# moonmath-ai/LiteAttention

Measured on AMD Instinct MI355X. Metric: self-attn TFLOPS + ms/step @ seq=75k d=128 bf16, sparsity 0->77%; 1/2/4/8 GPU, higher is better.
Workload: dtype bf16; 1 GPU; QK-Skip self-attention fwd, B=1 S=75600 H=40 D=128 bf16, imposed 42% sparsity (banded lists, thr=-inf), tiles 256x64; parallelism=heads sharded 1x40, launcher=single process

## Files before the change

### liteattention_amd/csrc/gen_blocks.py

```python
from gen_asm import *


def flush_block(flush_label, back_label, T, tail=None):
    label(flush_label)
    flush_domask(T[4], T[5])
    emit(f"s_add_u32 {s(S_DOWORD)}, {s(S_DOWORD)}, 4")
    emit(f"s_mov_b32 {s(S_BIT)}, 1")
    if tail:
        tail()
    else:
        emit("s_waitcnt lgkmcnt(0)")
    emit(f"s_branch {back_label}")


def inval_block(lbl, back, R):
    label(lbl)
    for qb in R.QBS:
        emit(f"v_mov_b32 {v(R.MLOC[qb])}, {v(R.NEGINF)}")
        emit(f"v_mov_b32 {v(R.NMS[qb])}, {v(R.NEGINF)}")
    emit(f"s_branch {back}")


def rescale_o_block(lbl, back, T, scaled, nops=2, tail=None):
    label(lbl)
# ... 96 lines not shown
    emit(f"s_cmp_eq_u32 {s(S_DOMASK)}, 0")
    emit(f"s_cbranch_scc1 {nofl}")
    flush_domask(T[4], T[5])
    label(nofl)
    for _ in range(nops):
        emit("s_nop 15")


def q_row_address(T, row):
    emit(f"v_min_i32 {v(T[3])}, {v(row)}, {s(S_T1)}")
    emit(f"v_mad_u64_u32 {vr(T[4], 2)}, {sr(S_T64)}, {v(T[3])}, {s(S_QRS)}, 0")
    emit(f"v_add_co_u32 {v(T[4])}, vcc, {v(T[4])}, {v(T[6])}")
    emit(f"v_addc_co_u32 {v(T[5])}, vcc, 0, {v(T[5])}, vcc")
    emit(f"v_add_co_u32 {v(T[4])}, vcc, {s(S_QBASE)}, {v(T[4])}")
    emit(f"v_mov_b32 {v(T[7])}, {s(S_QBASE + 1)}")
    emit(f"v_addc_co_u32 {v(T[5])}, vcc, {v(T[5])}, {v(T[7])}, vcc")


def q_rows_to_agprs(T, n_qb, n_frag, frag_bytes, q_a0, row_of, loaded=None):
    emit(f"v_lshlrev_b32 {v(T[6])}, 4, {v(T[0])}")
    for qb in range(n_qb):
        q_row_address(T, row_of(qb, False))
        for f in range(n_frag):
            emit(f"global_load_dwordx4 {vr(4 * n_frag * qb + 4 * f, 4)}, {vr(T[4], 2)}, off offset:{frag_bytes * f}")
    (loaded or (lambda: emit("s_waitcnt vmcnt(0)")))()
    for qb in range(n_qb):
        emit(f"v_cmp_gt_i32 vcc, {s(S_SEQLENQ)}, {v(row_of(qb, True))}")
        for r in range(4 * n_frag * qb, 4 * n_frag * (qb + 1)):
            emit(f"v_cndmask_b32 {v(r)}, 0, {v(r)}, vcc")
    for r in range(4 * n_frag * n_qb):
        emit(f"v_accvgpr_write_b32 a{q_a0 + r}, {v(r)}")


def zero_accumulators(regs):
    emit("; ---- state")
    for r in regs:
        emit(f"v_accvgpr_write_b32 a{r}, 0")


def read_tile_table(T, TABV):
    emit("; ---- tile addresses of positions 1..3 from the table; K(0) fragments -> AGPRs, S(0) = K(0) Q^T, then K(1) fragments")
    emit(f"v_mov_b32 {v(T[6])}, {s(S_TAB)}")
    emit(f"ds_read_b64 {vr(T[8], 2)}, {v(T[6])} offset:32")
    emit(f"ds_read_b64 {vr(T[10], 2)}, {v(T[6])} offset:48")
    emit(f"ds_read_b64 {vr(T[12], 2)}, {v(T[6])} offset:24")
    emit(f"v_add_u32 {v(TABV)}, 32, {v(T[6])}")


def k2_base(T):
    emit(("DRAIN",))
    emit(f"v_readfirstlane_b32 {s(TBS[0])}, {v(T[8])}")
    emit(f"v_readfirstlane_b32 {s(TBS[0] + 1)}, {v(T[9])}")


def stage_k2(k_ops, T):
    for it in k_ops:
        out.append(it)
        if "m0" in it:
            emit("s_nop 0")
    for dst, src in ((TBS[0], T[10]), (TBS[0] + 1, T[11]), (VBS[0], T[12]), (VBS[0] + 1, T[13])):
        emit(f"v_readfirstlane_b32 {s(dst)}, {v(src)}")


def mask_ops(T, NEGINF, lane_key, keys):
    for key, regs in keys:
        emit(f"v_add_u32 {v(T[0])}, {key}, {v(lane_key)}")
# ... 14 lines not shown
```

### liteattention_amd/csrc/gen_fwd_x64.py

```python
#!/usr/bin/env python
import os
import sys
from types import SimpleNamespace

from gen_asm import *
from gen_blocks import *
from gen_epilogue import store_epilogue

set_label_prefix(".LX")
OPT = options("LA_X64_OPT")
SCHEDULE_ONLY = {"snake", "x", "cap1", "cap2", "dmagaps", "dmapol", "align", "pad4", "pad4b", "e64", "wp2", "wp2b", "wc2", "kearly", "klate", "klate2", "expblock", "norot", "w2", "pk"}


DTYPE = os.environ.get("LA_X64_DTYPE", "bf16")
MFMA_OP = {"bf16": "v_mfma_f32_32x32x16_bf16", "f16": "v_mfma_f32_32x32x16_f16"}[DTYPE]
CVT_OP = {"bf16": "v_cvt_pk_bf16_f32", "f16": "v_cvt_pk_f16_f32"}[DTYPE]
W2 = "w2" in OPT
D = int(os.environ.get("LA_X64_D", "128"))
assert D in (64, 96, 128, 192, 256)
assert not W2 or D == 64
HALF = os.environ.get("LA_X64_FORM", "") == "half"
assert not HALF or (D in (64, 96, 128) and not W2)
DL = 64 if D == 64 else (128 if D <= 128 else 256)
NQB = 1 if W2 else (2 if DL <= 128 else 1)
# ... 656 lines not shown
        emit("s_waitcnt lgkmcnt(0)")
        w2_qk()
        w2_stats(first_tile=False, can_be_first=False)
        label(skip)
    w2_tail()


def prologue():
    stamp(0)
    read_params(LANE, T[0], [S_HSTRIDE] if HALF else [])
    if HALF:
        emit("; ---- half = wave >> 1: its vote words, its activity words; the window starts as positions [0, 64)")
        emit(f"s_lshr_b32 {s(S_T0)}, {s(S_WAVE)}, 1")
        emit(f"s_mul_i32 {s(S_T0)}, {s(S_T0)}, {s(S_HSTRIDE)}")
        emit(f"s_add_u32 {s(S_DOFLAGS)}, {s(S_DOFLAGS)}, {s(S_T0)}")
        emit(f"s_add_u32 {s(S_ACTPTR)}, {s(S_EXPORT)}, {s(S_T0)}")
        emit(f"v_mov_b32 {v(T[0])}, {s(S_ACTPTR)}")
        emit(f"ds_read_b64 {vr(T[4], 2)}, {v(T[0])}")
        emit("s_waitcnt lgkmcnt(0)")
        emit(f"v_readfirstlane_b32 {s(S_ACT)}, {v(T[4])}")
        emit(f"v_readfirstlane_b32 {s(S_ACT + 1)}, {v(T[5])}")
        emit(f"s_add_u32 {s(S_ACTPTR)}, {s(S_ACTPTR)}, 4")
    emit(f"s_mov_b32 {s(S_CC)}, {s(S_C)}")
    emit(f"s_mov_b32 {s(S_CC + 1)}, {s(S_C)}")
    emit(f"s_sub_u32 {s(S_NM1)}, {s(S_NTILES)}, 1")
    emit(f"s_lshl_b32 {s(S_DMAW)}, {s(S_WAVE)}, {ROW_SHIFT + (3 if W2 else 4)}")
    emit(f"s_add_u32 {s(S_DMAW)}, {s(S_DMAW)}, {s(S_LDS)}")
    emit(f"s_mov_b32 {s(S_I)}, 0")
    if DOTSUM:
        emit(f"s_mov_b32 {s(S_ONES)}, {ONES_BITS}")
    emit(f"s_mov_b32 {s(S_RESC)}, 0")
    emit(f"v_mov_b32 {v(NEGINF)}, 0xff800000")

    emit("; ---- per-lane constants")
    emit(f"v_lshrrev_b32 {v(T[0])}, 5, {v(LANE)}")
    emit(f"v_lshlrev_b32 {v(HH4)}, 2, {v(T[0])}")
    emit(f"v_and_b32 {v(T[1])}, 31, {v(LANE)}")
    emit(f"v_and_b32 {v(T[2])}, 15, {v(LANE)}")
    emit(f"v_lshlrev_b32 {v(T[3])}, {ROW_SHIFT}, {v(T[1])}")
    emit(f"v_add_u32 {v(T[3])}, {s(S_LDS)}, {v(T[3])}")
    if DL == 64:
        emit(f"v_lshrrev_b32 {v(T[8])}, 1, {v(T[1])}")
        emit(f"v_and_b32 {v(T[8])}, 7, {v(T[8])}")
    for ks in range(4 if DL == 64 else 8):
        emit(f"v_add_u32 {v(T[4])}, {2 * ks}, {v(T[0])}")
        emit(f"v_xor_b32 {v(T[4])}, {v(T[4])}, {v(T[8] if DL == 64 else T[2])}")
        emit(f"v_lshl_add_u32 {v(KADDR[ks])}, {v(T[4])}, 4, {v(T[3])}")
    emit(f"v_lshrrev_b32 {v(T[4])}, 2, {v(T[2])}")
    emit(f"v_add_u32 {v(T[5])}, {v(HH4)}, {v(T[4])}")
    emit(f"v_lshlrev_b32 {v(T[5])}, {ROW_SHIFT}, {v(T[5])}")
    emit(f"v_add_u32 {v(T[5])}, {s(S_LDS)}, {v(T[5])}")
    emit(f"v_add_u32 {v(T[5])}, {V_REGION}, {v(T[5])}")
    emit(f"v_lshrrev_b32 {v(T[6])}, 4, {v(LANE)}")
    emit(f"v_and_b32 {v(T[7])}, 1, {v(T[6])}")
    emit(f"v_lshlrev_b32 {v(T[7])}, 5, {v(T[7])}")
    emit(f"v_and_b32 {v(T[8])}, 3, {v(T[2])}")
    emit(f"v_lshl_or_b32 {v(T[7])}, {v(T[8])}, 3, {v(T[7])}")
    emit(f"v_add_u32 {v(T[5])}, {v(T[5])}, {v(T[7])}")
    if DL == 64:
        emit(f"v_lshrrev_b32 {v(T[4])}, 1, {v(T[4])}")
    for db in range(2 if DL == 64 else 4):
        emit(f"v_xor_b32 {v(T[7])}, {db}, {v(T[4])}")
        emit(f"v_lshl_add_u32 {v(VADDR[db])}, {v(T[7])}, 6, {v(T[5])}")
    emit(f"s_lshl_b32 {s(S_T0)}, {s(S_WAVE)}, {3 if W2 else 4}")
    if DL == 64:
        emit(f"v_lshrrev_b32 {v(T[6])}, 3, {v(LANE)}")
        emit(f"v_and_b32 {v(T[7])}, 7, {v(LANE)}")
        emit(f"v_add_u32 {v(RIPROW)}, {s(S_T0)}, {v(T[6])}")
        emit(f"v_lshrrev_b32 {v(T[8])}, 1, {v(T[6])}")
        emit(f"v_xor_b32 {v(RAGK)}, {v(T[7])}, {v(T[8])}")
        emit(f"v_lshlrev_b32 {v(RAGK)}, 4, {v(RAGK)}")
# ... 15 lines not shown
    else:
        emit(f"v_add_u32 {v(RIPROW)}, {s(S_T0)}, {v(T[0])}")
        emit(f"v_xor_b32 {v(RAGK)}, {v(T[1])}, {v(T[0])}")
        emit(f"v_lshlrev_b32 {v(RAGK)}, 4, {v(RAGK)}")
        emit(f"v_lshlrev_b32 {v(RAGV)}, 2, {v(T[0])}")
        emit(f"v_xor_b32 {v(RAGV)}, {v(T[1])}, {v(RAGV)}")
        emit(f"v_lshlrev_b32 {v(RAGV)}, 4, {v(RAGV)}")
    emit(f"s_mov_b32 {s(S_T1)}, {s(S_LASTROW)}")
    RSTEP = (64 // NW) // PW
    for j in range(PW):
        bias = DMA_BIAS - 1024 * (j & 3)
        emit(f"v_add_u32 {v(T[4])}, {RSTEP * j}, {v(RIPROW)}")
        emit(f"v_min_i32 {v(T[4])}, {v(T[4])}, {s(S_T1)}")
        emit(f"v_mul_lo_u32 {v(LK[j])}, {v(T[4])}, {s(S_KRS)}")
        def in_row(reg):
            if D != DL:
                emit(f"v_subrev_u32 {v(T[7])}, {2 * DL - 2 * D}, {v(reg)}")
                emit(f"v_cmp_le_u32 vcc, {2 * D}, {v(reg)}")
                emit(f"v_cndmask_b32 {v(reg)}, {v(reg)}, {v(T[7])}, vcc")
        emit(f"v_xor_b32 {v(T[5])}, {((RSTEP * j) >> (1 if DL == 64 else 0)) << 4}, {v(RAGK)}")
        in_row(T[5])
        emit(f"v_add_u32 {v(LK[j])}, {v(LK[j])}, {v(T[5])}")
        emit(f"v_mul_lo_u32 {v(LV[j])}, {v(T[4])}, {s(S_VRS)}")
        if D == 128 or D == 64:
            emit(f"v_add_u32 {v(LV[j])}, {v(LV[j])}, {v(RAGV)}")
        else:
            emit(f"v_xor_b32 {v(T[5])}, {((RSTEP * j) & 3) << 6}, {v(RAGV)}")
            in_row(T[5])
            emit(f"v_add_u32 {v(LV[j])}, {v(LV[j])}, {v(T[5])}")
        if bias:
            emit(f"v_add_u32 {v(LK[j])}, {bias}, {v(LK[j])}")
            emit(f"v_add_u32 {v(LV[j])}, {bias}, {v(LV[j])}")

    emit("; ---- Q fragments -> AGPRs: row q_row0 + 64*wave + 32*qb + l31, d = 16*ks + 8*hh; rows past seqlen_q are ZERO rows")
    emit(f"s_lshl_b32 {s(S_T0)}, {s(S_WAVE)}, {5 + NQB - 1}")
    emit(f"s_add_u32 {s(S_T0)}, {s(S_T0)}, {s(S_QROW0)}")
    emit(f"s_sub_u32 {s(S_T1)}, {s(S_SEQLENQ)}, 1")

    def q_row(qb, again):
        if not again:
            emit(f"v_add_u32 {v(QROW[qb])}, {s(S_T0)}, {v(T[1])}")
            if qb:
                emit(f"v_add_u32 {v(QROW[qb])}, 32, {v(QROW[qb])}")
        return QROW[qb]
    q_rows_to_agprs(T, NQB, KS, 32, Q_A0, q_row, loaded=lambda: (stamp(1), emit("s_waitcnt vmcnt(0)"), stamp(2)))
    zero_accumulators(range(16 * DB * NQB))
    for qb in range(NQB):
        emit(f"v_mov_b32 {v(MTRUE[qb])}, 0xff800000")
        emit(f"v_mov_b32 {v(L0[qb])}, 0")
        emit(f"v_mov_b32 {v(L1[qb])}, 0")
        emit(f"v_mov_b32 {v(ALPHA[qb])}, 1.0")
        if HALF:
            emit(f"v_mov_b32 {v(MREF[qb])}, 0xff800000")
            emit(f"v_mov_b32 {v(MTHR[qb])}, 0xff800000")
            emit(f"v_mov_b32 {v(NMS[qb])}, 0")

    if W2:
        emit("; ---- w2: K(0) fragments -> AGPRs")
        emit(f"v_mov_b32 {v(TABV)}, {s(S_TAB)}")
        emit(f"v_add_u32 {v(TABV)}, 16, {v(TABV)}")
        for j in range(NKF):
            emit(k_read(0, j))
        emit(f"s_mov_b32 {s(S_DOMASK)}, 0")
        emit(f"s_mov_b32 {s(S_BIT)}, 1")
        emit(f"s_mov_b32 {s(S_DOWORD)}, {s(S_DOFLAGS)}")
        emit(("DRAIN",))
        emit("s_barrier")
        return
    read_tile_table(T, TABV)
    for j in range(NKF):
        emit(k_read(0, j))
    k2_base(T)
    ord1 = [(f & 1) * KS + (f >> 1) for f in range(NKF)]
    if HALF:
        noqk0 = new_label("noqk0")
        emit(f"s_bitcmp1_b32 {s(S_ACT)}, 0")
        emit(f"s_cbranch_scc0 {noqk0}")
    for t in range(NG):
        out.append(mfma_qk(0, ord1[t // NQB], qb_of(t)))
    if HALF:
        label(noqk0)
    for j in range(NKF):
        emit(k_read(KV_TILE, j))
    emit(("DRAIN",))
    emit("s_barrier")
    stage_k2(dma_ops(0, 0, do_k=True, do_v=False), T)
    emit("s_nop 7")
    if HALF:
# ... 139 lines not shown
```

### liteattention_amd/csrc/la_fwd_common.h

```cpp
#pragma once
#include <hip/hip_runtime.h>
#include <stdint.h>

#include "la_kernel_params.h"

namespace la {

typedef __bf16 bf16x8 __attribute__((ext_vector_type(8)));
typedef short s16x4 __attribute__((ext_vector_type(4)));
typedef short s16x8 __attribute__((ext_vector_type(8)));
typedef float f32x16 __attribute__((ext_vector_type(16)));
typedef float f32x8 __attribute__((ext_vector_type(8)));
typedef unsigned int u32x2 __attribute__((ext_vector_type(2)));
typedef unsigned int u32x4 __attribute__((ext_vector_type(4)));

typedef _Float16 f16x8 __attribute__((ext_vector_type(8)));
typedef _Float16 f16x4 __attribute__((ext_vector_type(4)));
typedef __bf16 bf16x4 __attribute__((ext_vector_type(4)));
typedef float f32x4 __attribute__((ext_vector_type(4)));

template <bool F16> struct Elem16;
template <> struct Elem16<false> {
    typedef bf16x8 x8;
    typedef bf16x4 x4;
// ... 77 lines not shown
        if (!((live[pos >> 5] >> (pos & 31)) & 1u)) continue;
        const int n = seq[pos];
        const bool raw_skip = !first && !((doflags[pos >> 5] >> (pos & 31)) & 1u);
        first = false;
        bool skip = raw_skip;
        if (has_md && skip) {
            if (md.end > n && md.has_more()) { md.advance(); md.load(k_tiles); }
            const bool must_do = n <= md.start && n > md.end;
            skip = skip && !must_do;
        }
        if (skip != is_skipping) {
            if (w <= k_tiles) write_row[w] = static_cast<ListT>(n);
            ++w;
            is_skipping = skip;
        }
        if ((endflags[pos >> 5] >> (pos & 31)) & 1u) {
            is_skipping = true;
            if (!raw_skip) { if (w <= k_tiles) write_row[w] = static_cast<ListT>(n); ++w; }
        }
    }
    write_row[0] = static_cast<ListT>(min(w - 1, k_tiles));
}

__device__ __forceinline__ int wave_inclusive_scan(int v) {
    v += __builtin_amdgcn_update_dpp(0, v, 0x111, 0xf, 0xf, true);
    v += __builtin_amdgcn_update_dpp(0, v, 0x112, 0xf, 0xf, true);
    v += __builtin_amdgcn_update_dpp(0, v, 0x114, 0xf, 0xf, true);
    v += __builtin_amdgcn_update_dpp(0, v, 0x118, 0xf, 0xf, true);
    v += __builtin_amdgcn_update_dpp(0, v, 0x142, 0xa, 0xf, false);
    v += __builtin_amdgcn_update_dpp(0, v, 0x143, 0xc, 0xf, false);
    return v;
}

template <typename ListT>
__device__ __forceinline__ void write_skip_list_wave(const int* seq, const unsigned* endflags, const unsigned* doflags,
                                                     int n_tiles, ListT* __restrict__ write_row,
                                                     const int* __restrict__ must_do_row, int k_tiles, int lane) {
    int md_start = 0, md_end = 0;
    if (must_do_row != nullptr) {
        if (must_do_row[0] > 2) {
            if (lane == 0) write_skip_list(seq, endflags, doflags, n_tiles, write_row, must_do_row, k_tiles);
            return;
        }
        md_start = must_do_row[1];
        md_end = must_do_row[2];
    }
    int w = 1;
    int carry_skip = 1;
    for (int base = 0; base < n_tiles; base += 64) {
        const int pos = base + lane;
        const bool live = pos < n_tiles;
        int n = 0;
        bool raw = false, is_end = false;
        if (live) {
            n = seq[pos];
            raw = pos != 0 && !((doflags[pos >> 5] >> (pos & 31)) & 1u);
            is_end = (endflags[pos >> 5] >> (pos & 31)) & 1u;
        }
        const bool skip = raw && !(n <= md_start && n > md_end);
        const unsigned long long after_b = __ballot(live && (is_end || skip));
        const unsigned long long below = (1ull << lane) - 1ull;
        const int before = lane == 0 ? carry_skip : static_cast<int>((after_b >> ((lane - 1) & 63)) & 1ull);
        const bool e1 = live && (static_cast<int>(skip) != before);
        const bool e2 = live && is_end && !raw;
        const unsigned long long e1_b = __ballot(e1), e2_b = __ballot(e2);
        int slot = w + __popcll(e1_b & below) + __popcll(e2_b & below);
        if (e1) { if (slot <= k_tiles) write_row[slot] = static_cast<ListT>(n); ++slot; }
        if (e2) { if (slot <= k_tiles) write_row[slot] = static_cast<ListT>(n); }
        w += __popcll(e1_b) + __popcll(e2_b);
        carry_skip = static_cast<int>((after_b >> 63) & 1ull);
    }
    if (lane == 0) write_row[0] = static_cast<ListT>(min(w - 1, k_tiles));
}

template <typename ListT>
__device__ __forceinline__ void write_skip_list_wave_live(const int* seq, const unsigned* endflags, const unsigned* doflags,
                                                          const unsigned* livebits, int n_tiles, ListT* __restrict__ write_row,
                                                          const int* __restrict__ must_do_row, int k_tiles, int lane) {
    int md_start = 0, md_end = 0;
    if (must_do_row != nullptr) {
        if (must_do_row[0] > 2) {
            if (lane == 0) write_skip_list_live(seq, endflags, doflags, livebits, n_tiles, write_row, must_do_row, k_tiles);
            return;
        }
        md_start = must_do_row[1];
        md_end = must_do_row[2];
    }
    int w = 1, carry_skip = 1;
    bool seen = false;
    for (int base = 0; base < n_tiles; base += 64) {
        const int pos = base + lane;
        const bool live = pos < n_tiles && ((livebits[pos >> 5] >> (pos & 31)) & 1u);
        const unsigned long long live_b = __ballot(live);
        const unsigned long long below = (1ull << lane) - 1ull;
        const unsigned long long lb = live_b & below;
        int n = 0;
        bool raw = false, is_end = false;
        if (live) {
            n = seq[pos];
            const bool first = !seen && lb == 0ull;
            raw = !first && !((doflags[pos >> 5] >> (pos & 31)) & 1u);
            is_end = (endflags[pos >> 5] >> (pos & 31)) & 1u;
        }
        const bool skip = raw && !(n <= md_start && n > md_end);
        const unsigned long long after_b = __ballot(live && (is_end || skip));
        const int before = lb != 0ull ? static_cast<int>((after_b >> (63 - __clzll(static_cast<long long>(lb)))) & 1ull) : carry_skip;
        const bool e1 = live && (static_cast<int>(skip) != before);
        const bool e2 = live && is_end && !raw;
        const unsigned long long e1_b = __ballot(e1), e2_b = __ballot(e2);
        int slot = w + __popcll(e1_b & below) + __popcll(e2_b & below);
        if (e1) { if (slot <= k_tiles) write_row[slot] = static_cast<ListT>(n); ++slot; }
        if (e2) { if (slot <= k_tiles) write_row[slot] = static_cast<ListT>(n); }
        w += __popcll(e1_b) + __popcll(e2_b);
        if (live_b != 0ull) {
            carry_skip = static_cast<int>((after_b >> (63 - __clzll(static_cast<long long>(live_b)))) & 1ull);
            seen = true;
        }
    }
    if (lane == 0) write_row[0] = static_cast<ListT>(min(w - 1, k_tiles));
}

__device__ __forceinline__ void store_empty_rows(const FwdParams& p, const SeqView& sv, int h, int row0, int nrows, int head_dim,
                                                 int tid, int nthreads) {
    const int chunks = head_dim / 8;
    const int rows = min(nrows, sv.seqlen_q - row0);
    for (int base = 0; base < rows * chunks; base += nthreads) {
        const int i = base + tid;
        if (i >= rows * chunks) continue;
        const int r = row0 + i / chunks, ch = i % chunks;
        const u32x4 z = {0u, 0u, 0u, 0u};
        *reinterpret_cast<u32x4*>(p.o + sv.o_off + static_cast<int64_t>(r) * p.o_row_stride + h * p.o_head_stride + ch * 8) = z;
        if (p.lse != nullptr && ch == 0) sv.lse_row0[r] = INFINITY;
    }
}

template <int C = 64>
__device__ __forceinline__ int xcd_work_id() {
    const int bid = blockIdx.x, nwg = gridDim.x;
    const int full = (nwg / (8 * C)) * (8 * C);
    if (bid >= full) return bid;
    const int xcd = bid & 7, idx = bid >> 3;
    return ((idx / C) * 8 + xcd) * C + (idx % C);
}

__device__ __forceinline__ void work_item(const FwdParams& p, int vid, int& bh, int& m_block) {
    const int cnt = p.q_tile_count;
// ... 175 lines not shown
```

### liteattention_amd/csrc/la_fwd_kernel_x64.hip

```cpp
#include <hip/hip_runtime.h>
#include <stdint.h>

#include "la_fwd_common.h"

#ifndef LA_X64_M16
#define LA_X64_M16 0
#endif
#ifndef LA_X64_BODY_INC
#define LA_X64_BODY_INC "la_fwd_x64_body.inc"
#endif
#ifndef LA_X64_F16_BODY_INC
#define LA_X64_F16_BODY_INC "la_fwd_x64_f16_body.inc"
#endif
#ifndef LA_X64_HALF_BODY_INC
#define LA_X64_HALF_BODY_INC "la_fwd_x64_half_body.inc"
#endif
#ifndef LA_X64_HALF_F16_BODY_INC
#define LA_X64_HALF_F16_BODY_INC "la_fwd_x64_half_f16_body.inc"
#endif
#ifndef LA_X64_D64_HALF_BODY_INC
#define LA_X64_D64_HALF_BODY_INC "la_fwd_x64_d64_half_body.inc"
#endif
#ifndef LA_X64_D64_HALF_F16_BODY_INC
#define LA_X64_D64_HALF_F16_BODY_INC "la_fwd_x64_d64_half_f16_body.inc"
// ... 288 lines not shown
        }
    } else if (SKIPABLE) {
        if (!pre) {
            for (int base = 0; base < 2 * words; base += NT)
                if (base + tid < 2 * words) doflags[base + tid] = 0u;
            __syncthreads();
            if (wave == 0) {
                int n;
                LA_WITH_LIST_TYPE(p.list_int16, n = expand_read_list(static_cast<const ListT*>(p.read_list) + list_off, seq, endflags, k_tiles, lane));
                if (lane == 0) { walk_n[0] = n; walk_n[1] = k_tiles; }
            } else if (dynamic && tid == 64) {
                meta[3] = next_work_item(p, LA_SCHED_C, &meta[2]);
            }
        }
    } else {
        for (int base = 0; base < 2 * words; base += NT)
            if (base + tid < 2 * words) doflags[base + tid] = 0u;
        for (int base = 0; base < k_tiles; base += NT)
            if (base + tid < k_tiles) seq[base + tid] = k_tiles - 1 - (base + tid);
        if (tid == 0) walk_n[0] = k_tiles;
    }
    __syncthreads();
    if (!SKIPABLE && dynamic && tid == 64) meta[3] = next_work_item(p, LA_SCHED_C, &meta[2]);
    LA_PHASE_STAMP(2);
    const int n_tiles = walk_n[0];
    if (kOverlap && pre && tid == 64) meta[3] = meta[4];

    const unsigned char* const kg = reinterpret_cast<const unsigned char*>(p.k + k_off + hk * p.k_head_stride);
    const unsigned char* const vg = reinterpret_cast<const unsigned char*>(p.v + v_off + hk * p.v_head_stride);
    const unsigned char* const qg = reinterpret_cast<const unsigned char*>(p.q + q_off + h * p.q_head_stride);
    const int k_rs = static_cast<int>(p.k_row_stride * 2), v_rs = static_cast<int>(p.v_row_stride * 2);
    const int last_row = seqlen_k - 1;

    if (tid == 0) {
        auto lds_addr = [](const void* ptr) { return static_cast<unsigned>(reinterpret_cast<uintptr_t>(LDS_PTR(const unsigned char, ptr))); };
        const uint64_t kb64 = reinterpret_cast<uint64_t>(kg), vb64 = reinterpret_cast<uint64_t>(vg), qb64 = reinterpret_cast<uint64_t>(qg);
        param[0] = static_cast<unsigned>(kb64); param[1] = static_cast<unsigned>(kb64 >> 32);
        param[2] = static_cast<unsigned>(vb64); param[3] = static_cast<unsigned>(vb64 >> 32);
        param[4] = k_rs; param[5] = v_rs; param[6] = last_row; param[7] = n_tiles;
        param[8] = __float_as_uint(p.scale_log2); param[9] = __float_as_uint(p.thr);
        param[10] = seqlen_k - (k_tiles - 1) * X_BN; param[11] = seq[0] == k_tiles - 1 ? 1u : 0u;
        param[12] = lds_addr(tab); param[13] = lds_addr(doflags);
        param[14] = static_cast<unsigned>(qb64); param[15] = static_cast<unsigned>(qb64 >> 32);
        param[16] = static_cast<unsigned>(p.q_row_stride * 2); param[17] = m_block * BM; param[18] = seqlen_q;
        param[19] = HALF ? lds_addr(doflags + 4 * words) : 0u;
        param[20] = lds_addr(smem); param[21] = __float_as_uint(-p.scale_log2);
        param[22] = __float_as_uint(p.rescale_tau / p.scale_log2);
        param[23] = HALF ? static_cast<unsigned>(hbw * 4) : 0u;
        const uint64_t ob64 = reinterpret_cast<uint64_t>(p.o + o_off + h * p.o_head_stride);
        const uint64_t lb64 = p.lse != nullptr ? reinterpret_cast<uint64_t>(lse_row0) : 0ull;
        param[24] = static_cast<unsigned>(ob64); param[25] = static_cast<unsigned>(ob64 >> 32);
        param[26] = static_cast<unsigned>(p.o_row_stride * 2);
        param[27] = __float_as_uint(p.scale_log2 * 0.69314718055994530942f);
        param[28] = static_cast<unsigned>(lb64); param[29] = static_cast<unsigned>(lb64 >> 32);
        param[30] = __float_as_uint(1.0f); param[31] = __float_as_uint(0.0f);
    }

    {
        constexpr int kDmaBias = 3072;
        const int saferow = max(last_row - (X_BN - 1), 0);
        const uint64_t kb = reinterpret_cast<uint64_t>(kg) - kDmaBias, vb = reinterpret_cast<uint64_t>(vg) - kDmaBias;
        for (int base = 0; base < n_tiles + 4; base += NT) {
            const int i = base + tid;
            if (i >= n_tiles + 4) continue;
            const int row = min(seq[min(i, n_tiles - 1)] * X_BN, saferow);
            tab[2 * i] = kb + static_cast<uint64_t>(row) * static_cast<uint64_t>(k_rs);
            tab[2 * i + 1] = vb + static_cast<uint64_t>(row) * static_cast<uint64_t>(v_rs);
        }
    }

    {
        const int rip = lane / (X_ROW / 16), cpos = lane % (X_ROW / 16);
        auto in_row = [](int chunk) { return chunk >= D / 8 ? chunk - (DL - D) / 8 : chunk; };
        auto dma_tile = [&](int n, bool do_k, int kbuf, bool do_v, int vbuf) {
#pragma unroll
            for (int j = 0; j < PIECES; ++j) {
                const int r = (X_BN / NW) * wave + RPP * j + rip;
                const int grow = min(n * X_BN + r, last_row);
                const int k_swz = DL == 64 ? ((r >> 1) & 7) : (r & 15);
                const int v_swz = DL == 64 ? (((r >> 1) & 1) << 2) : ((LA_X64_M16 != 0 && D == 128) ? ((r & 7) << 1) : ((r & 3) << 2));
                if (do_k) x_dma16(kg + static_cast<int64_t>(grow) * k_rs + (in_row(cpos ^ k_swz) << 4),
                                  k_lds + kbuf * X_TILE + (PIECES * wave + j) * 1024);
                if (do_v) x_dma16(vg + static_cast<int64_t>(grow) * v_rs + (in_row(cpos ^ v_swz) << 4),
                                  k_lds + 2 * X_TILE + vbuf * X_TILE + (PIECES * wave + j) * 1024);
            }
        };
        const int n0 = seq[0], n1 = seq[min(1, n_tiles - 1)];
        dma_tile(n0, true, 0, true, 0);
        dma_tile(n1, true, 1, false, 0);
    }
    __syncthreads();
    LA_PHASE_STAMP(3);

    {
        const unsigned param_addr = __builtin_amdgcn_readfirstlane(
            static_cast<unsigned>(reinterpret_cast<uintptr_t>(LDS_PTR(unsigned, param))));
        const int wave_s = wave;
        if constexpr (HALF && D == 64 && F16) {
            asm volatile(
#include LA_X64_D64_HALF_F16_BODY_INC
                : : "s"(wave_s), "s"(param_addr) : LA_X64_CLOBBERS);
        } else if constexpr (HALF && D == 64) {
            asm volatile(
#include LA_X64_D64_HALF_BODY_INC
                : : "s"(wave_s), "s"(param_addr) : LA_X64_CLOBBERS);
        } else if constexpr (HALF && D == 96 && F16) {
            asm volatile(
#include LA_X64_D96_HALF_F16_BODY_INC
                : : "s"(wave_s), "s"(param_addr) : LA_X64_CLOBBERS);
        } else if constexpr (HALF && D == 96) {
            asm volatile(
#include LA_X64_D96_HALF_BODY_INC
                : : "s"(wave_s), "s"(param_addr) : LA_X64_CLOBBERS);
        } else if constexpr (HALF && F16) {
            asm volatile(
#include LA_X64_HALF_F16_BODY_INC
                : : "s"(wave_s), "s"(param_addr) : LA_X64_CLOBBERS);
        } else if constexpr (HALF) {
            asm volatile(
#include LA_X64_HALF_BODY_INC
                : : "s"(wave_s), "s"(param_addr) : LA_X64_CLOBBERS);
        } else if constexpr (D == 64 && F16 && x_two_waves_per_simd(D)) {
            asm volatile(
// ... 198 lines not shown
```

### liteattention_amd/csrc/la_fwd_kernel_x64_fp8.hip

```cpp
#include <hip/hip_runtime.h>
#include <stdint.h>

#include "la_fwd_common.h"

#ifndef LA_X64F8_BODY_INC
#define LA_X64F8_BODY_INC "la_fwd_x64_fp8_body.inc"
#endif
#ifndef LA_X64F8_EXP_BODY_INC
#define LA_X64F8_EXP_BODY_INC "la_fwd_x64_fp8_exp_body.inc"
#endif
#ifndef LA_X64F8_LVALU_BODY_INC
#define LA_X64F8_LVALU_BODY_INC "la_fwd_x64_fp8_lvalu_body.inc"
#endif

#ifndef LA_X64F8_CONSTS_INC
#define LA_X64F8_CONSTS_INC "la_fwd_x64_fp8_consts.h"
#endif
#ifndef LA_X64F8_EXP_CONSTS_INC
#define LA_X64F8_EXP_CONSTS_INC "la_fwd_x64_fp8_exp_consts.h"
#endif
#ifndef LA_X64F8_LVALU_CONSTS_INC
#define LA_X64F8_LVALU_CONSTS_INC "la_fwd_x64_fp8_lvalu_consts.h"
#endif
#ifndef LA_X64F8_D64_BODY_INC
// ... 196 lines not shown
                if (base + tid < 2 * words) doflags[base + tid] = 0u;
            __syncthreads();
            if (wave == 0) {
                int n;
                LA_WITH_LIST_TYPE(p.list_int16, n = expand_read_list(static_cast<const ListT*>(p.read_list) + list_off, seq, endflags, k_tiles, lane));
                if (lane == 0) { walk_n[0] = n; walk_n[1] = k_tiles; }
            } else if (dynamic && tid == 64) {
                meta[3] = next_work_item(p, LA_SCHED_C, &meta[2]);
            }
        }
    } else {
        for (int base = 0; base < 2 * words; base += 256)
            if (base + tid < 2 * words) doflags[base + tid] = 0u;
        for (int base = 0; base < k_tiles; base += 256)
            if (base + tid < k_tiles) seq[base + tid] = k_tiles - 1 - (base + tid);
        if (tid == 0) walk_n[0] = k_tiles;
    }
    __syncthreads();
    if (!SKIPABLE && dynamic && tid == 64) meta[3] = next_work_item(p, LA_SCHED_C, &meta[2]);
    const int n_tiles = walk_n[0];
    if (kOverlap && pre && tid == 64) meta[3] = meta[4];

    const unsigned char* const kg = reinterpret_cast<const unsigned char*>(p.k) + k_off + hk * p.k_head_stride;
    const unsigned char* const vg = reinterpret_cast<const unsigned char*>(p.v) +
                                    (static_cast<int64_t>(b) * (p.num_heads / p.h_ratio) + hk) * p.k_tiles * kTileBytes;
    const unsigned char* const qg = reinterpret_cast<const unsigned char*>(p.q) + q_off + h * p.q_head_stride;
    const int k_rs = static_cast<int>(p.k_row_stride), v_rs = 0;
    const float qd = p.q_descale ? p.q_descale[b * p.q_descale_batch_stride + hk * p.q_descale_head_stride] : 1.f;
    const float kd = p.k_descale ? p.k_descale[b * p.k_descale_batch_stride + hk * p.k_descale_head_stride] : 1.f;
    const float vd = p.v_descale ? p.v_descale[b * p.v_descale_batch_stride + hk * p.v_descale_head_stride] : 1.f;
    const float c = p.scale_log2 * qd * kd;
    const int last_row = seqlen_k - 1;

    if (tid == 0) {
        auto lds_addr = [](const void* ptr) { return static_cast<unsigned>(reinterpret_cast<uintptr_t>(LDS_PTR(const unsigned char, ptr))); };
        const uint64_t kb64 = reinterpret_cast<uint64_t>(kg), vb64 = reinterpret_cast<uint64_t>(vg), qb64 = reinterpret_cast<uint64_t>(qg);
        param[0] = static_cast<unsigned>(kb64); param[1] = static_cast<unsigned>(kb64 >> 32);
        param[2] = static_cast<unsigned>(vb64); param[3] = static_cast<unsigned>(vb64 >> 32);
        param[4] = k_rs; param[5] = v_rs; param[6] = last_row; param[7] = n_tiles;
        param[8] = __float_as_uint(c); param[9] = __float_as_uint(p.thr);
        param[10] = seqlen_k - (k_tiles - 1) * X_BN; param[11] = seq[0] == k_tiles - 1 ? 1u : 0u;
        param[12] = lds_addr(tab); param[13] = lds_addr(doflags);
        param[14] = static_cast<unsigned>(qb64); param[15] = static_cast<unsigned>(qb64 >> 32);
        param[16] = static_cast<unsigned>(p.q_row_stride); param[17] = m_block * kRows; param[18] = seqlen_q;
        param[19] = 0; param[20] = lds_addr(smem); param[21] = __float_as_uint(-c);
        param[22] = __float_as_uint(X_TAU[PMODE] / c);
        const uint64_t ob64 = reinterpret_cast<uint64_t>(p.o + o_off + h * p.o_head_stride);
        const uint64_t lb64 = p.lse != nullptr ? reinterpret_cast<uint64_t>(lse_row0) : 0ull;
        param[24] = static_cast<unsigned>(ob64); param[25] = static_cast<unsigned>(ob64 >> 32);
        param[26] = static_cast<unsigned>(p.o_row_stride * 2);
        param[27] = __float_as_uint(c * 0.69314718055994530942f);
        param[28] = static_cast<unsigned>(lb64); param[29] = static_cast<unsigned>(lb64 >> 32);
        param[30] = __float_as_uint(vd); param[31] = __float_as_uint(-X_OFFSET[PMODE] * 0.69314718055994530942f);
    }

    {
        constexpr int kDmaBias = kWide ? 3072 : 1024;
        const int saferow = max(last_row - (X_BN - 1), 0);
        const uint64_t kb = reinterpret_cast<uint64_t>(kg) - kDmaBias, vb = reinterpret_cast<uint64_t>(vg);
        for (int base = 0; base < n_tiles + 4; base += 256) {
            const int i = base + tid;
            if (i >= n_tiles + 4) continue;
            const int n = seq[min(i, n_tiles - 1)];
            tab[2 * i] = kb + static_cast<uint64_t>(min(n * X_BN, saferow)) * static_cast<uint64_t>(k_rs);
            tab[2 * i + 1] = vb + static_cast<uint64_t>(n) * kTileBytes;
        }
    }

    {
        const int rip = lane >> 3, cpos = lane & 7;
        auto dma_k = [&](int n, int kbuf) {
            if constexpr (kWide) {
                const int rip16 = lane >> 4, cpos16 = lane & 15;
#pragma unroll
                for (int j = 0; j < 4; ++j) {
                    const int r = 16 * wave + 4 * j + rip16;
                    const int grow = min(n * X_BN + r, last_row);
                    const int cs = min(cpos16 ^ (r & 15), D / 16 - 1);
                    xf8_dma16(kg + static_cast<int64_t>(grow) * k_rs + (cs << 4), k_lds + kbuf * X_TILE + (4 * wave + j) * 1024);
                }
            } else if constexpr (D == 64) {
                const int R = 8 * wave + rip;
                const int cs = cpos ^ ((R >> 1) & 7);
                const int grow = min(n * X_BN + R + 32 * (cs >> 2), last_row);
                xf8_dma16(kg + static_cast<int64_t>(grow) * k_rs + ((cs & 3) << 4), k_lds + kbuf * X_TILE + wave * 1024);
            } else {
#pragma unroll
                for (int j = 0; j < 2; ++j) {
                    const int r = 16 * wave + 8 * j + rip;
                    const int grow = min(n * X_BN + r, last_row);
                    const int cs = min(cpos ^ ((r >> 1) & 7), D / 16 - 1);
                    xf8_dma16(kg + static_cast<int64_t>(grow) * k_rs + (cs << 4), k_lds + kbuf * X_TILE + (2 * wave + j) * 1024);
                }
            }
        };
        const int n0 = seq[0], n1 = seq[min(1, n_tiles - 1)];
        dma_k(n0, 0);
        constexpr int kPieces = kTileBytes / 4096;
#pragma unroll
        for (int j = 0; j < kPieces; ++j)
            xf8_dma16(vg + static_cast<int64_t>(n0) * kTileBytes + (kPieces * wave + j) * 1024 + lane * 16,
                      k_lds + 2 * X_TILE + (kPieces * wave + j) * 1024);
        dma_k(n1, 1);
    }
    __syncthreads();

    {
        const unsigned param_addr = __builtin_amdgcn_readfirstlane(
            static_cast<unsigned>(reinterpret_cast<uintptr_t>(LDS_PTR(unsigned, param))));
        const int wave_s = wave;
        if constexpr (D == 256 && PMODE == 2) {
            asm volatile(
#include LA_X64F8_D256_LVALU_BODY_INC
                : : "s"(wave_s), "s"(param_addr) : LA_X64F8_CLOBBERS);
        } else if constexpr (D == 256 && PMODE == 1) {
            asm volatile(
#include LA_X64F8_D256_EXP_BODY_INC
                : : "s"(wave_s), "s"(param_addr) : LA_X64F8_CLOBBERS);
        } else if constexpr (D == 256) {
            asm volatile(
#include LA_X64F8_D256_BODY_INC
                : : "s"(wave_s), "s"(param_addr) : LA_X64F8_CLOBBERS);
        } else if constexpr (D == 192 && PMODE == 2) {
            asm volatile(
#include LA_X64F8_D192_LVALU_BODY_INC
                : : "s"(wave_s), "s"(param_addr) : LA_X64F8_CLOBBERS);
        } else if constexpr (D == 192 && PMODE == 1) {
            asm volatile(
#include LA_X64F8_D192_EXP_BODY_INC
                : : "s"(wave_s), "s"(param_addr) : LA_X64F8_CLOBBERS);
        } else if constexpr (D == 192) {
            asm volatile(
#include LA_X64F8_D192_BODY_INC
                : : "s"(wave_s), "s"(param_addr) : LA_X64F8_CLOBBERS);
        } else if constexpr (D == 96 && PMODE == 2) {
            asm volatile(
#include LA_X64F8_D96_LVALU_BODY_INC
// ... 116 lines not shown
```

Measured before the change: 1335 TFLOP/s (executed: FLOPs of listed tiles only).

## Overlap prologue Q and K/V loads with setup, widen skip-list writer

Q fragments are now loaded straight into AGPRs early, so per-lane constant setup and accumulator zeroing run while the loads are in flight. The ragged-row zeroing becomes a branch that runs only for partial tiles. The initial K/V tile DMAs in the bf16 and fp8 kernels are issued before the parameter and table writes, so those writes hide load latency. The skip-list writer now handles four positions per lane with a wave scan instead of several ballots per 64 positions, which cuts loop iterations but adds per-lane serial work.

```diff
diff --git a/liteattention_amd/csrc/gen_blocks.py b/liteattention_amd/csrc/gen_blocks.py
--- a/liteattention_amd/csrc/gen_blocks.py
+++ b/liteattention_amd/csrc/gen_blocks.py
@@ -152,6 +152,31 @@
         emit(f"v_accvgpr_write_b32 a{q_a0 + r}, {v(r)}")
 
 
+def q_loads_to_agprs(T, n_qb, n_frag, frag_bytes, q_a0, row_of):
+    emit(f"v_lshlrev_b32 {v(T[6])}, 4, {v(T[0])}")
+    for qb in range(n_qb):
+        q_row_address(T, row_of(qb, False))
+        for f in range(n_frag):
+            emit(f"global_load_dwordx4 {ar(q_a0 + 4 * n_frag * qb + 4 * f, 4)}, {vr(T[4], 2)}, off offset:{frag_bytes * f}")
+
+
+def q_rows_ragged_fix(T, n_qb, n_frag, q_a0, row_of):
+    for qb in range(n_qb):
+        full = new_label("qfull")
+        emit(f"v_cmp_gt_i32 vcc, {s(S_SEQLENQ)}, {v(row_of(qb, True))}")
+        emit("s_cmp_eq_u64 vcc, -1")
+        emit(f"s_cbranch_scc1 {full}")
+        base = q_a0 + 4 * n_frag * qb
+        for r0 in range(base, base + 4 * n_frag, 8):
+            for k in range(8):
+                emit(f"v_accvgpr_read_b32 {v(T[k])}, a{r0 + k}")
+            for k in range(8):
+                emit(f"v_cndmask_b32 {v(T[k])}, 0, {v(T[k])}, vcc")
+            for k in range(8):
+                emit(f"v_accvgpr_write_b32 a{r0 + k}, {v(T[k])}")
+        label(full)
+
+
 def zero_accumulators(regs):
     emit("; ---- state")
     for r in regs:
diff --git a/liteattention_amd/csrc/gen_fwd_x64.py b/liteattention_amd/csrc/gen_fwd_x64.py
--- a/liteattention_amd/csrc/gen_fwd_x64.py
+++ b/liteattention_amd/csrc/gen_fwd_x64.py
@@ -712,11 +712,25 @@
     emit(f"s_mov_b32 {s(S_RESC)}, 0")
     emit(f"v_mov_b32 {v(NEGINF)}, 0xff800000")
 
-    emit("; ---- per-lane constants")
+    emit("; ---- per-lane constants the Q addresses need")
     emit(f"v_lshrrev_b32 {v(T[0])}, 5, {v(LANE)}")
     emit(f"v_lshlrev_b32 {v(HH4)}, 2, {v(T[0])}")
     emit(f"v_and_b32 {v(T[1])}, 31, {v(LANE)}")
     emit(f"v_and_b32 {v(T[2])}, 15, {v(LANE)}")
+    emit("; ---- Q fragments -> AGPRs: row q_row0 + 64*wave + 32*qb + l31, d = 16*ks + 8*hh; rows past seqlen_q are ZERO rows")
+    emit(f"s_lshl_b32 {s(S_T0)}, {s(S_WAVE)}, {5 + NQB - 1}")
+    emit(f"s_add_u32 {s(S_T0)}, {s(S_T0)}, {s(S_QROW0)}")
+    emit(f"s_sub_u32 {s(S_T1)}, {s(S_SEQLENQ)}, 1")
+
+    def q_row(qb, again):
+        if not again:
+            emit(f"v_add_u32 {v(QROW[qb])}, {s(S_T0)}, {v(T[1])}")
+            if qb:
+                emit(f"v_add_u32 {v(QROW[qb])}, 32, {v(QROW[qb])}")
+        return QROW[qb]
+    q_loads_to_agprs(T, NQB, KS, 32, Q_A0, q_row)
+    stamp(1)
+    emit("; ---- per-lane constants (under the Q loads)")
     emit(f"v_lshlrev_b32 {v(T[3])}, {ROW_SHIFT}, {v(T[1])}")
     emit(f"v_add_u32 {v(T[3])}, {s(S_LDS)}, {v(T[3])}")
     if DL == 64:
@@ -798,18 +812,6 @@
             emit(f"v_add_u32 {v(LK[j])}, {bias}, {v(LK[j])}")
             emit(f"v_add_u32 {v(LV[j])}, {bias}, {v(LV[j])}")
 
-    emit("; ---- Q fragments -> AGPRs: row q_row0 + 64*wave + 32*qb + l31, d = 16*ks + 8*hh; rows past seqlen_q are ZERO rows")
-    emit(f"s_lshl_b32 {s(S_T0)}, {s(S_WAVE)}, {5 + NQB - 1}")
-    emit(f"s_add_u32 {s(S_T0)}, {s(S_T0)}, {s(S_QROW0)}")
-    emit(f"s_sub_u32 {s(S_T1)}, {s(S_SEQLENQ)}, 1")
-
-    def q_row(qb, again):
-        if not again:
-            emit(f"v_add_u32 {v(QROW[qb])}, {s(S_T0)}, {v(T[1])}")
-            if qb:
-                emit(f"v_add_u32 {v(QROW[qb])}, 32, {v(QROW[qb])}")
-        return QROW[qb]
-    q_rows_to_agprs(T, NQB, KS, 32, Q_A0, q_row, loaded=lambda: (stamp(1), emit("s_waitcnt vmcnt(0)"), stamp(2)))
     zero_accumulators(range(16 * DB * NQB))
     for qb in range(NQB):
         emit(f"v_mov_b32 {v(MTRUE[qb])}, 0xff800000")
@@ -820,6 +822,9 @@
             emit(f"v_mov_b32 {v(MREF[qb])}, 0xff800000")
             emit(f"v_mov_b32 {v(MTHR[qb])}, 0xff800000")
             emit(f"v_mov_b32 {v(NMS[qb])}, 0")
+    emit("s_waitcnt vmcnt(0)")
+    stamp(2)
+    q_rows_ragged_fix(T, NQB, KS, Q_A0, q_row)
 
     if W2:
         emit("; ---- w2: K(0) fragments -> AGPRs")
diff --git a/liteattention_amd/csrc/la_fwd_common.h b/liteattention_amd/csrc/la_fwd_common.h
--- a/liteattention_amd/csrc/la_fwd_common.h
+++ b/liteattention_amd/csrc/la_fwd_common.h
@@ -133,10 +133,12 @@
     return v;
 }
 
+constexpr int LIST_WRITER_WIDTH = 4;
 template <typename ListT>
 __device__ __forceinline__ void write_skip_list_wave(const int* seq, const unsigned* endflags, const unsigned* doflags,
                                                      int n_tiles, ListT* __restrict__ write_row,
                                                      const int* __restrict__ must_do_row, int k_tiles, int lane) {
+    constexpr int W = LIST_WRITER_WIDTH;
     int md_start = 0, md_end = 0;
     if (must_do_row != nullptr) {
         if (must_do_row[0] > 2) {
@@ -148,27 +150,41 @@
     }
     int w = 1;
     int carry_skip = 1;
-    for (int base = 0; base < n_tiles; base += 64) {
-        const int pos = base + lane;
-        const bool live = pos < n_tiles;
-        int n = 0;
-        bool raw = false, is_end = false;
-        if (live) {
-            n = seq[pos];
-            raw = pos != 0 && !((doflags[pos >> 5] >> (pos & 31)) & 1u);
-            is_end = (endflags[pos >> 5] >> (pos & 31)) & 1u;
-        }
-        const bool skip = raw && !(n <= md_start && n > md_end);
-        const unsigned long long after_b = __ballot(live && (is_end || skip));
-        const unsigned long long below = (1ull << lane) - 1ull;
-        const int before = lane == 0 ? carry_skip : static_cast<int>((after_b >> ((lane - 1) & 63)) & 1ull);
-        const bool e1 = live && (static_cast<int>(skip) != before);
-        const bool e2 = live && is_end && !raw;
-        const unsigned long long e1_b = __ballot(e1), e2_b = __ballot(e2);
-        int slot = w + __popcll(e1_b & below) + __popcll(e2_b & below);
-        if (e1) { if (slot <= k_tiles) write_row[slot] = static_cast<ListT>(n); ++slot; }
-        if (e2) { if (slot <= k_tiles) write_row[slot] = static_cast<ListT>(n); }
-        w += __popcll(e1_b) + __popcll(e2_b);
+    for (int base = 0; base < n_tiles; base += 64 * W) {
+        const int pos0 = base + W * lane;
+        unsigned do_w = 0u, end_w = 0u;
+        if (pos0 < n_tiles) { do_w = doflags[pos0 >> 5] >> (pos0 & 31); end_w = endflags[pos0 >> 5] >> (pos0 & 31); }
+        int n[W];
+        bool live[W], raw[W], is_end[W], skip[W];
+        bool after = false;
+#pragma unroll
+        for (int j = 0; j < W; ++j) {
+            live[j] = pos0 + j < n_tiles;
+            n[j] = live[j] ? seq[pos0 + j] : 0;
+            raw[j] = live[j] && pos0 + j != 0 && !((do_w >> j) & 1u);
+            is_end[j] = live[j] && ((end_w >> j) & 1u);
+            skip[j] = raw[j] && !(n[j] <= md_start && n[j] > md_end);
+            after = live[j] && (is_end[j] || skip[j]);
+        }
+        const unsigned long long after_b = __ballot(after);
+        int before = lane == 0 ? carry_skip : static_cast<int>((after_b >> ((lane - 1) & 63)) & 1ull);
+        bool e1[W], e2[W];
+        int cnt = 0;
+#pragma unroll
+        for (int j = 0; j < W; ++j) {
+            e1[j] = live[j] && (static_cast<int>(skip[j]) != before);
+            e2[j] = is_end[j] && !raw[j];
+            before = (is_end[j] || skip[j]) ? 1 : 0;
+            cnt += static_cast<int>(e1[j]) + static_cast<int>(e2[j]);
+        }
+        const int incl = wave_inclusive_scan(cnt);
+        int slot = w + incl - cnt;
+#pragma unroll
+        for (int j = 0; j < W; ++j) {
+            if (e1[j]) { if (slot <= k_tiles) write_row[slot] = static_cast<ListT>(n[j]); ++slot; }
+            if (e2[j]) { if (slot <= k_tiles) write_row[slot] = static_cast<ListT>(n[j]); ++slot; }
+        }
+        w += __builtin_amdgcn_readlane(incl, 63);
         carry_skip = static_cast<int>((after_b >> 63) & 1ull);
     }
     if (lane == 0) write_row[0] = static_cast<ListT>(min(w - 1, k_tiles));
@@ -178,6 +194,7 @@
 __device__ __forceinline__ void write_skip_list_wave_live(const int* seq, const unsigned* endflags, const unsigned* doflags,
                                                           const unsigned* livebits, int n_tiles, ListT* __restrict__ write_row,
                                                           const int* __restrict__ must_do_row, int k_tiles, int lane) {
+    constexpr int W = LIST_WRITER_WIDTH;
     int md_start = 0, md_end = 0;
     if (must_do_row != nullptr) {
         if (must_do_row[0] > 2) {
@@ -189,30 +206,50 @@
     }
     int w = 1, carry_skip = 1;
     bool seen = false;
-    for (int base = 0; base < n_tiles; base += 64) {
-        const int pos = base + lane;
-        const bool live = pos < n_tiles && ((livebits[pos >> 5] >> (pos & 31)) & 1u);
-        const unsigned long long live_b = __ballot(live);
+    for (int base = 0; base < n_tiles; base += 64 * W) {
+        const int pos0 = base + W * lane;
+        unsigned do_w = 0u, end_w = 0u, live_w = 0u;
+        if (pos0 < n_tiles) {
+            do_w = doflags[pos0 >> 5] >> (pos0 & 31); end_w = endflags[pos0 >> 5] >> (pos0 & 31); live_w = livebits[pos0 >> 5] >> (pos0 & 31);
+        }
+        bool live[W];
+        bool any_live = false;
+#pragma unroll
+        for (int j = 0; j < W; ++j) { live[j] = pos0 + j < n_tiles && ((live_w >> j) & 1u); any_live = any_live || live[j]; }
+        const unsigned long long live_b = __ballot(any_live);
         const unsigned long long below = (1ull << lane) - 1ull;
         const unsigned long long lb = live_b & below;
-        int n = 0;
-        bool raw = false, is_end = false;
-        if (live) {
-            n = seq[pos];
-            const bool first = !seen && lb == 0ull;
-            raw = !first && !((doflags[pos >> 5] >> (pos & 31)) & 1u);
-            is_end = (endflags[pos >> 5] >> (pos & 31)) & 1u;
-        }
-        const bool skip = raw && !(n <= md_start && n > md_end);
-        const unsigned long long after_b = __ballot(live && (is_end || skip));
-        const int before = lb != 0ull ? static_cast<int>((after_b >> (63 - __clzll(static_cast<long long>(lb)))) & 1ull) : carry_skip;
-        const bool e1 = live && (static_cast<int>(skip) != before);
-        const bool e2 = live && is_end && !raw;
-        const unsigned long long e1_b = __ballot(e1), e2_b = __ballot(e2);
-        int slot = w + __popcll(e1_b & below) + __popcll(e2_b & below);
-        if (e1) { if (slot <= k_tiles) write_row[slot] = static_cast<ListT>(n); ++slot; }
-        if (e2) { if (slot <= k_tiles) write_row[slot] = static_cast<ListT>(n); }
-        w += __popcll(e1_b) + __popcll(e2_b);
+        bool first = !seen && lb == 0ull;
+        int n[W];
+        bool raw[W], is_end[W], skip[W];
+        bool after = false;
+#pragma unroll
+        for (int j = 0; j < W; ++j) {
+            n[j] = live[j] ? seq[pos0 + j] : 0;
+            raw[j] = live[j] && !first && !((do_w >> j) & 1u);
+            is_end[j] = live[j] && ((end_w >> j) & 1u);
+            skip[j] = raw[j] && !(n[j] <= md_start && n[j] > md_end);
+            if (live[j]) { after = is_end[j] || skip[j]; first = false; }
+        }
+        const unsigned long long after_b = __ballot(after);
+        int before = lb != 0ull ? static_cast<int>((after_b >> (63 - __clzll(static_cast<long long>(lb)))) & 1ull) : carry_skip;
+        bool e1[W], e2[W];
+        int cnt = 0;
+#pragma unroll
+        for (int j = 0; j < W; ++j) {
+            e1[j] = live[j] && (static_cast<int>(skip[j]) != before);
+            e2[j] = is_end[j] && !raw[j];
+            if (live[j]) before = (is_end[j] || skip[j]) ? 1 : 0;
+            cnt += static_cast<int>(e1[j]) + static_cast<int>(e2[j]);
+        }
+        const int incl = wave_inclusive_scan(cnt);
+        int slot = w + incl - cnt;
+#pragma unroll
+        for (int j = 0; j < W; ++j) {
+            if (e1[j]) { if (slot <= k_tiles) write_row[slot] = static_cast<ListT>(n[j]); ++slot; }
+            if (e2[j]) { if (slot <= k_tiles) write_row[slot] = static_cast<ListT>(n[j]); ++slot; }
+        }
+        w += __builtin_amdgcn_readlane(incl, 63);
         if (live_b != 0ull) {
             carry_skip = static_cast<int>((after_b >> (63 - __clzll(static_cast<long long>(live_b)))) & 1ull);
             seen = true;
diff --git a/liteattention_amd/csrc/la_fwd_kernel_x64.hip b/liteattention_amd/csrc/la_fwd_kernel_x64.hip
--- a/liteattention_amd/csrc/la_fwd_kernel_x64.hip
+++ b/liteattention_amd/csrc/la_fwd_kernel_x64.hip
@@ -344,6 +344,26 @@
     const int k_rs = static_cast<int>(p.k_row_stride * 2), v_rs = static_cast<int>(p.v_row_stride * 2);
     const int last_row = seqlen_k - 1;
 
+    {
+        const int rip = lane / (X_ROW / 16), cpos = lane % (X_ROW / 16);
+        auto in_row = [](int chunk) { return chunk >= D / 8 ? chunk - (DL - D) / 8 : chunk; };
+        auto dma_tile = [&](int n, bool do_k, int kbuf, bool do_v, int vbuf) {
+#pragma unroll
+            for (int j = 0; j < PIECES; ++j) {
+                const int r = (X_BN / NW) * wave + RPP * j + rip;
+                const int grow = min(n * X_BN + r, last_row);
+                const int k_swz = DL == 64 ? ((r >> 1) & 7) : (r & 15);
+                const int v_swz = DL == 64 ? (((r >> 1) & 1) << 2) : ((LA_X64_M16 != 0 && D == 128) ? ((r & 7) << 1) : ((r & 3) << 2));
+                if (do_k) x_dma16(kg + static_cast<int64_t>(grow) * k_rs + (in_row(cpos ^ k_swz) << 4),
+                                  k_lds + kbuf * X_TILE + (PIECES * wave + j) * 1024);
+                if (do_v) x_dma16(vg + static_cast<int64_t>(grow) * v_rs + (in_row(cpos ^ v_swz) << 4),
+                                  k_lds + 2 * X_TILE + vbuf * X_TILE + (PIECES * wave + j) * 1024);
+            }
+        };
+        const int n0 = seq[0], n1 = seq[min(1, n_tiles - 1)];
+        dma_tile(n0, true, 0, true, 0);
+        dma_tile(n1, true, 1, false, 0);
+    }
     if (tid == 0) {
         auto lds_addr = [](const void* ptr) { return static_cast<unsigned>(reinterpret_cast<uintptr_t>(LDS_PTR(const unsigned char, ptr))); };
         const uint64_t kb64 = reinterpret_cast<uint64_t>(kg), vb64 = reinterpret_cast<uint64_t>(vg), qb64 = reinterpret_cast<uint64_t>(qg);
@@ -381,26 +401,6 @@
         }
     }
 
-    {
-        const int rip = lane / (X_ROW / 16), cpos = lane % (X_ROW / 16);
-        auto in_row = [](int chunk) { return chunk >= D / 8 ? chunk - (DL - D) / 8 : chunk; };
-        auto dma_tile = [&](int n, bool do_k, int kbuf, bool do_v, int vbuf) {
-#pragma unroll
-            for (int j = 0; j < PIECES; ++j) {
-                const int r = (X_BN / NW) * wave + RPP * j + rip;
-                const int grow = min(n * X_BN + r, last_row);
-                const int k_swz = DL == 64 ? ((r >> 1) & 7) : (r & 15);
-                const int v_swz = DL == 64 ? (((r >> 1) & 1) << 2) : ((LA_X64_M16 != 0 && D == 128) ? ((r & 7) << 1) : ((r & 3) << 2));
-                if (do_k) x_dma16(kg + static_cast<int64_t>(grow) * k_rs + (in_row(cpos ^ k_swz) << 4),
-                                  k_lds + kbuf * X_TILE + (PIECES * wave + j) * 1024);
-                if (do_v) x_dma16(vg + static_cast<int64_t>(grow) * v_rs + (in_row(cpos ^ v_swz) << 4),
-                                  k_lds + 2 * X_TILE + vbuf * X_TILE + (PIECES * wave + j) * 1024);
-            }
-        };
-        const int n0 = seq[0], n1 = seq[min(1, n_tiles - 1)];
-        dma_tile(n0, true, 0, true, 0);
-        dma_tile(n1, true, 1, false, 0);
-    }
     __syncthreads();
     LA_PHASE_STAMP(3);
 
diff --git a/liteattention_amd/csrc/la_fwd_kernel_x64_fp8.hip b/liteattention_amd/csrc/la_fwd_kernel_x64_fp8.hip
--- a/liteattention_amd/csrc/la_fwd_kernel_x64_fp8.hip
+++ b/liteattention_amd/csrc/la_fwd_kernel_x64_fp8.hip
@@ -252,41 +252,6 @@
     const float c = p.scale_log2 * qd * kd;
     const int last_row = seqlen_k - 1;
 
-    if (tid == 0) {
-        auto lds_addr = [](const void* ptr) { return static_cast<unsigned>(reinterpret_cast<uintptr_t>(LDS_PTR(const unsigned char, ptr))); };
-        const uint64_t kb64 = reinterpret_cast<uint64_t>(kg), vb64 = reinterpret_cast<uint64_t>(vg), qb64 = reinterpret_cast<uint64_t>(qg);
-        param[0] = static_cast<unsigned>(kb64); param[1] = static_cast<unsigned>(kb64 >> 32);
-        param[2] = static_cast<unsigned>(vb64); param[3] = static_cast<unsigned>(vb64 >> 32);
-        param[4] = k_rs; param[5] = v_rs; param[6] = last_row; param[7] = n_tiles;
-        param[8] = __float_as_uint(c); param[9] = __float_as_uint(p.thr);
-        param[10] = seqlen_k - (k_tiles - 1) * X_BN; param[11] = seq[0] == k_tiles - 1 ? 1u : 0u;
-        param[12] = lds_addr(tab); param[13] = lds_addr(doflags);
-        param[14] = static_cast<unsigned>(qb64); param[15] = static_cast<unsigned>(qb64 >> 32);
-        param[16] = static_cast<unsigned>(p.q_row_stride); param[17] = m_block * kRows; param[18] = seqlen_q;
-        param[19] = 0; param[20] = lds_addr(smem); param[21] = __float_as_uint(-c);
-        param[22] = __float_as_uint(X_TAU[PMODE] / c);
-        const uint64_t ob64 = reinterpret_cast<uint64_t>(p.o + o_off + h * p.o_head_stride);
-        const uint64_t lb64 = p.lse != nullptr ? reinterpret_cast<uint64_t>(lse_row0) : 0ull;
-        param[24] = static_cast<unsigned>(ob64); param[25] = static_cast<unsigned>(ob64 >> 32);
-        param[26] = static_cast<unsigned>(p.o_row_stride * 2);
-        param[27] = __float_as_uint(c * 0.69314718055994530942f);
-        param[28] = static_cast<unsigned>(lb64); param[29] = static_cast<unsigned>(lb64 >> 32);
-        param[30] = __float_as_uint(vd); param[31] = __float_as_uint(-X_OFFSET[PMODE] * 0.69314718055994530942f);
-    }
-
-    {
-        constexpr int kDmaBias = kWide ? 3072 : 1024;
-        const int saferow = max(last_row - (X_BN - 1), 0);
-        const uint64_t kb = reinterpret_cast<uint64_t>(kg) - kDmaBias, vb = reinterpret_cast<uint64_t>(vg);
-        for (int base = 0; base < n_tiles + 4; base += 256) {
-            const int i = base + tid;
-            if (i >= n_tiles + 4) continue;
-            const int n = seq[min(i, n_tiles - 1)];
-            tab[2 * i] = kb + static_cast<uint64_t>(min(n * X_BN, saferow)) * static_cast<uint64_t>(k_rs);
-            tab[2 * i + 1] = vb + static_cast<uint64_t>(n) * kTileBytes;
-        }
-    }
-
     {
         const int rip = lane >> 3, cpos = lane & 7;
         auto dma_k = [&](int n, int kbuf) {
@@ -323,6 +288,41 @@
                       k_lds + 2 * X_TILE + (kPieces * wave + j) * 1024);
         dma_k(n1, 1);
     }
+    if (tid == 0) {
+        auto lds_addr = [](const void* ptr) { return static_cast<unsigned>(reinterpret_cast<uintptr_t>(LDS_PTR(const unsigned char, ptr))); };
+        const uint64_t kb64 = reinterpret_cast<uint64_t>(kg), vb64 = reinterpret_cast<uint64_t>(vg), qb64 = reinterpret_cast<uint64_t>(qg);
+        param[0] = static_cast<unsigned>(kb64); param[1] = static_cast<unsigned>(kb64 >> 32);
+        param[2] = static_cast<unsigned>(vb64); param[3] = static_cast<unsigned>(vb64 >> 32);
+        param[4] = k_rs; param[5] = v_rs; param[6] = last_row; param[7] = n_tiles;
+        param[8] = __float_as_uint(c); param[9] = __float_as_uint(p.thr);
+        param[10] = seqlen_k - (k_tiles - 1) * X_BN; param[11] = seq[0] == k_tiles - 1 ? 1u : 0u;
+        param[12] = lds_addr(tab); param[13] = lds_addr(doflags);
+        param[14] = static_cast<unsigned>(qb64); param[15] = static_cast<unsigned>(qb64 >> 32);
+        param[16] = static_cast<unsigned>(p.q_row_stride); param[17] = m_block * kRows; param[18] = seqlen_q;
+        param[19] = 0; param[20] = lds_addr(smem); param[21] = __float_as_uint(-c);
+        param[22] = __float_as_uint(X_TAU[PMODE] / c);
+        const uint64_t ob64 = reinterpret_cast<uint64_t>(p.o + o_off + h * p.o_head_stride);
+        const uint64_t lb64 = p.lse != nullptr ? reinterpret_cast<uint64_t>(lse_row0) : 0ull;
+        param[24] = static_cast<unsigned>(ob64); param[25] = static_cast<unsigned>(ob64 >> 32);
+        param[26] = static_cast<unsigned>(p.o_row_stride * 2);
+        param[27] = __float_as_uint(c * 0.69314718055994530942f);
+        param[28] = static_cast<unsigned>(lb64); param[29] = static_cast<unsigned>(lb64 >> 32);
+        param[30] = __float_as_uint(vd); param[31] = __float_as_uint(-X_OFFSET[PMODE] * 0.69314718055994530942f);
+    }
+
+    {
+        constexpr int kDmaBias = kWide ? 3072 : 1024;
+        const int saferow = max(last_row - (X_BN - 1), 0);
+        const uint64_t kb = reinterpret_cast<uint64_t>(kg) - kDmaBias, vb = reinterpret_cast<uint64_t>(vg);
+        for (int base = 0; base < n_tiles + 4; base += 256) {
+            const int i = base + tid;
+            if (i >= n_tiles + 4) continue;
+            const int n = seq[min(i, n_tiles - 1)];
+            tab[2 * i] = kb + static_cast<uint64_t>(min(n * X_BN, saferow)) * static_cast<uint64_t>(k_rs);
+            tab[2 * i + 1] = vb + static_cast<uint64_t>(n) * kTileBytes;
+        }
+    }
+
     __syncthreads();
 
     {
```

Result: no change. 1336 TFLOP/s (executed: FLOPs of listed tiles only) (median of 6 runs) (+0.1%).
